# zxhuang1698/ZeroShape

Measured on AMD Instinct MI355X. Metric: sdf_query_points_per_sec_vox128, higher is better.
Workload: dtype f16x3

## Files before the change

zeroshape_amd/build.py:

```python
import hashlib
import os
import subprocess
import sys

HERE = os.path.dirname(os.path.abspath(__file__))
CSRC = os.path.join(HERE, "csrc")
INCLUDE = os.path.join(os.path.dirname(HERE), "include")
LIB = os.path.join(HERE, "libzeroshape_hip.so")
OBJDIR = os.path.join(HERE, "csrc", "_obj")

ARCH = "gfx950"
COMMON = ["--offload-arch=" + ARCH, "-O3", "-std=c++17", "-fPIC", "-Wall",
          "-Wno-unused-function", "-I", INCLUDE]
EXTRA = {
    "chamfer.hip": ["-ffp-contract=off", "-fno-slp-vectorize"],
    "chamfer_grid.hip": ["-ffp-contract=off"],
    "pose_search.hip": ["-ffp-contract=off"],
    "sdf_decoder_split.hip": ["-fno-slp-vectorize", "-fno-honor-nans", "-mllvm", "-amdgpu-mfma-vgpr-form"],
    "marching_cubes.hip": ["-ffp-contract=off"],
    "render.hip": ["-ffp-contract=off"],
    "attn_vis.hip": ["-ffp-contract=off"],
    "seen_mesh.hip": ["-ffp-contract=off"],
    "mesh_weld.hip": ["-ffp-contract=off"],
    "field_normals.hip": ["-ffp-contract=off"],
    "mesh_components.hip": ["-ffp-contract=off"],
    "mesh_colors.hip": ["-ffp-contract=off"],
    "mesh_smooth.hip": ["-ffp-contract=off"],
    "mesh_simplify.hip": ["-ffp-contract=off"],
    "mesh_distance.hip": ["-ffp-contract=off"],
}


def sources():
    return sorted(f for f in os.listdir(CSRC) if f.endswith(".hip"))


def _includes(path, seen):
    import re
    with open(path, "rb") as fh:
        text = fh.read().decode("utf-8", "replace")
    for name in re.findall(r'^\s*#\s*include\s+["<]([^">]+)[">]', text, flags=re.M):
        for base in (os.path.dirname(path), INCLUDE):
            f = os.path.normpath(os.path.join(base, name))
            if os.path.exists(f):
                if f not in seen:
                    seen.append(f)
                    _includes(f, seen)
                break
    return seen


def _stamp(src, flags):
    h = hashlib.sha1()
    h.update(" ".join(os.path.relpath(f, HERE) if os.path.isabs(f) else f for f in flags).encode())
    for f in [src] + sorted(_includes(src, [])):
        with open(f, "rb") as fh:
            h.update(fh.read())
    return h.hexdigest()


def build(force=False, verbose=False):
    hipcc = os.environ.get("HIPCC", "/opt/rocm/bin/hipcc")
    os.makedirs(OBJDIR, exist_ok=True)
    objs, rebuilt = [], False
    for name in sources():
        src = os.path.join(CSRC, name)
        obj = os.path.join(OBJDIR, name[:-4] + ".o")
        flags = COMMON + EXTRA.get(name, [])
        stamp_file = obj + ".stamp"
        stamp = _stamp(src, flags)
        old = open(stamp_file).read() if os.path.exists(stamp_file) else ""
        if force or not os.path.exists(obj) or old != stamp:
            cmd = [hipcc] + flags + ["-c", src, "-o", obj]
            if verbose:
                print(" ".join(cmd), flush=True)
            subprocess.check_call(cmd)
            with open(stamp_file, "w") as fh:
                fh.write(stamp)
            rebuilt = True
        objs.append(obj)
    if rebuilt or not os.path.exists(LIB):
        cmd = [hipcc, "--offload-arch=" + ARCH, "-shared", "-fPIC", "-o", LIB] + objs
        if verbose:
            print(" ".join(cmd), flush=True)
        subprocess.check_call(cmd)
    return LIB


if __name__ == "__main__":
    print(build(force="--force" in sys.argv, verbose="--verbose" in sys.argv or "-v" in sys.argv))
```

zeroshape_amd/csrc/sdf_prologue.hip:

```cpp
#include "zs_common.h"
#include "sdf_layout.h"
#include "../../include/zeroshape_hip.h"

#include <math.h>

namespace {

using namespace zs::lay;

constexpr int ROWS = 4;
constexpr int LIN_THREADS = 256;
constexpr int KMAX = 1024;

__device__ __forceinline__ float wave_sum(float v) {
#pragma unroll
    for (int o = 32; o > 0; o >>= 1) v += __shfl_xor(v, o, 64);
    return v;
}

__device__ __forceinline__ float erf_ref(float x) { return erff(x); }

template <bool LN_IN, bool GELU, bool RESID, bool POS>
__global__ __launch_bounds__(LIN_THREADS) void lat_linear_kernel(
    const float *__restrict__ X, int ldx, size_t x_stride, int K, const float *__restrict__ Wt,
    const float *__restrict__ bias, int N, const float *__restrict__ ln_g,
    const float *__restrict__ ln_b, const float *__restrict__ resid, int ldr, size_t r_stride,
    const float *__restrict__ pos, float *__restrict__ Y, int ldy, size_t y_stride, int rows) {
    __shared__ float xs[ROWS][KMAX];
    const int img = blockIdx.z;
    const int r0 = blockIdx.x * ROWS;
    const int n = blockIdx.y * LIN_THREADS + threadIdx.x;
    X += (size_t)img * x_stride;
    Y += (size_t)img * y_stride;

    for (int i = threadIdx.x; i < ROWS * K; i += LIN_THREADS) {
        const int r = i / K, k = i - r * K;
        const int rr = min(r0 + r, rows - 1);
        xs[r][k] = X[(size_t)rr * ldx + k];
    }
    __syncthreads();
    if (LN_IN) {
        const int w = threadIdx.x >> 6, lane = threadIdx.x & 63;
        float v[4], s = 0.f;
#pragma unroll
        for (int j = 0; j < 4; j++) {
            v[j] = xs[w][lane + 64 * j];
            s += v[j];
        }
        const float mean = wave_sum(s) * (1.0f / 256.0f);
        float q = 0.f;
#pragma unroll
        for (int j = 0; j < 4; j++) {
            const float d = v[j] - mean;
            q = fmaf(d, d, q);
        }
        const float rstd = 1.0f / sqrtf(wave_sum(q) * (1.0f / 256.0f) + 1e-6f);
#pragma unroll
        for (int j = 0; j < 4; j++) {
            const int k = lane + 64 * j;
            xs[w][k] = fmaf((v[j] - mean) * rstd, ln_g[k], ln_b[k]);
        }
        __syncthreads();
    }
    float acc[ROWS];
#pragma unroll
    for (int r = 0; r < ROWS; r++) acc[r] = 0.f;
    for (int k0 = 0; k0 < K; k0 += 16) {
        float w[16];
#pragma unroll
        for (int j = 0; j < 16; j++) w[j] = Wt[(size_t)(k0 + j) * N + n];
#pragma unroll
        for (int j = 0; j < 16; j++)
#pragma unroll
            for (int r = 0; r < ROWS; r++) acc[r] = fmaf(xs[r][k0 + j], w[j], acc[r]);
    }
    const float b = bias[n];
#pragma unroll
    for (int r = 0; r < ROWS; r++) {
        const int row = r0 + r;
        if (row >= rows) break;
        float v = acc[r] + b;
        if (POS) v += pos[(size_t)row * N + n];
        if (GELU) v = 0.5f * v * (1.0f + erf_ref(v * 0.70710678118654752440f));
        if (RESID) v += resid[(size_t)img * r_stride + (size_t)row * ldr + n];
        Y[(size_t)row * ldy + n] = v;
    }
}

__global__ __launch_bounds__(256) void lat_self_attn_kernel(const float *__restrict__ qkv,
                                                            size_t stride, float *__restrict__ out,
                                                            size_t out_stride) {
    __shared__ float ks[L][HD];
    __shared__ float vs[L][HD];
    const int hd = blockIdx.x, img = blockIdx.y;
    qkv += (size_t)img * stride;
    out += (size_t)img * out_stride;
    for (int i = threadIdx.x; i < L * HD; i += 256) {
        const int r = i / HD, d = i - r * HD;
        ks[r][d] = qkv[(size_t)r * (3 * C) + C + hd * HD + d];
        vs[r][d] = qkv[(size_t)r * (3 * C) + 2 * C + hd * HD + d];
    }
    __syncthreads();
    const int i = threadIdx.x;
    if (i >= L) return;
    float q[HD], o[HD];
#pragma unroll
    for (int d = 0; d < HD; d++) {
        q[d] = qkv[(size_t)i * (3 * C) + hd * HD + d];
        o[d] = 0.f;
    }
    const float scale = 0.17677669529663688110f;
    float m = -INFINITY, z = 0.f;
    for (int j = 0; j < L; j++) {
        float s = 0.f;
#pragma unroll
        for (int d = 0; d < HD; d++) s = fmaf(q[d], ks[j][d], s);
        s *= scale;
        const float mn = fmaxf(m, s);
        const float a = expf(m - mn), p = expf(s - mn);
        z = fmaf(z, a, p);
#pragma unroll
        for (int d = 0; d < HD; d++) o[d] = fmaf(p, vs[j][d], o[d] * a);
        m = mn;
    }
    const float inv = 1.0f / z;
#pragma unroll
    for (int d = 0; d < HD; d++) out[(size_t)i * C + hd * HD + d] = o[d] * inv;
}

__global__ __launch_bounds__(256) void pack_kv_kernel(const float *__restrict__ scratch,
                                                      size_t scratch_stride,
                                                      float *__restrict__ programs,
                                                      size_t program_stride) {
    const int img = blockIdx.y;
    const int e = blockIdx.x * 256 + threadIdx.x;
    const int lane = e & 63;
    const int r = (e >> 6) & 15;
    const int which = (e >> 10) & 1;
    int t = e >> 11;
    const int lt = t % LT;
    t /= LT;
    const int hd = t & 7;
    const int blk = t >> 3;
    if (blk >= BLOCKS) return;
    const float *sc = scratch + (size_t)img * scratch_stride;
    const int rw = (r & 3) + 8 * (r >> 2) + 4 * (lane >> 5);
    const int lrow = 32 * lt + (which == 0 ? (lane & 31) : rw);
    const int dim = which == 0 ? rw : (lane & 31);
    float val = 0.f;
    if (lrow < L) {
        if (blk == 0)
            val = sc[S_QKV0 + (size_t)lrow * (3 * C) + (1 + which) * C + hd * HD + dim];
        else
            val = sc[S_KV1 + (size_t)lrow * (2 * C) + which * C + hd * HD + dim];
    }
    const int group = blk * G_BLOCK + hd * G_HEAD + G_QKV_HEAD + lt * 8 + which * 4 + (r >> 2);
    programs[(size_t)img * program_stride + (size_t)group * GROUP_FLOATS + lane * 4 + (r & 3)] = val;
}

template <bool LN_IN, bool GELU, bool RESID, bool POS>
void launch_linear(hipStream_t s, int batch, const float *X, int ldx, size_t x_stride, int K,
                   const float *Wt, const float *bias, int N, const float *g, const float *b,
                   const float *resid, int ldr, size_t r_stride, const float *pos, float *Y, int ldy,
                   size_t y_stride) {
    dim3 grid((L + ROWS - 1) / ROWS, N / LIN_THREADS, batch);
    hipLaunchKernelGGL((lat_linear_kernel<LN_IN, GELU, RESID, POS>), grid, dim3(LIN_THREADS), 0, s, X,
                       ldx, x_stride, K, Wt, bias, N, g, b, resid, ldr, r_stride, pos, Y, ldy,
                       y_stride, L);
}

}

__global__ __launch_bounds__(256) void verdict_stats_kernel(const float *__restrict__ got, const float *__restrict__ want, int m,
                                                            float band, float tol, float tol_occ, float *__restrict__ stats,
                                                            int *__restrict__ flags) {
    __shared__ float red[4][256];
    __shared__ int redi[2][256];
    const int b = blockIdx.x, t = threadIdx.x;
    const float *g = got + (size_t)b * m, *w = want + (size_t)b * m;
    float mx = 0.f, sum = 0.f, mw = 0.f, mo = 0.f;
    int flips = 0, bad = 0;
    for (int i = t; i < m; i += 256) {
        const float x = g[i], y = w[i];
        if (!isfinite(x) || !isfinite(y)) bad = 1;
        const float d = fabsf(x - y);
        mx = fmaxf(mx, d);
        sum += d;
        mw = fmaxf(mw, fabsf(y));
        mo = fmaxf(mo, fabsf(1.0f / (1.0f + expf(-x)) - 1.0f / (1.0f + expf(-y))));
        flips += ((x > 0.f) != (y > 0.f)) && fabsf(y) >= band;
    }
    red[0][t] = mx; red[1][t] = sum; red[2][t] = mw; red[3][t] = mo;
    redi[0][t] = flips; redi[1][t] = bad;
    __syncthreads();
    for (int o = 128; o > 0; o >>= 1) {
        if (t < o) {
            red[0][t] = fmaxf(red[0][t], red[0][t + o]);
            red[1][t] += red[1][t + o];
            red[2][t] = fmaxf(red[2][t], red[2][t + o]);
            red[3][t] = fmaxf(red[3][t], red[3][t + o]);
            redi[0][t] += redi[0][t + o];
            redi[1][t] |= redi[1][t + o];
        }
        __syncthreads();
    }
    if (t == 0) {
        const bool finite = redi[1][0] == 0;
        const float nan = __builtin_bit_cast(float, 0x7fc00000u);
        float *o = stats + (size_t)b * 5;
        o[0] = finite ? red[0][0] : nan;
        o[1] = finite ? red[1][0] / (float)m : nan;
        o[2] = finite ? red[2][0] : nan;
        o[3] = finite ? red[3][0] : nan;
        o[4] = (float)redi[0][0];
        if (flags) {
            flags[2 * b] = (finite && red[0][0] <= tol) ? 0 : 1;
            flags[2 * b + 1] = (finite && red[3][0] <= tol_occ && redi[0][0] == 0) ? 0 : 1;
        }
    }
}

extern "C" int zs_sdf_verdict_stats(const float *got, const float *want, int batch, int m, float flip_band, float tol,
                                    float tol_occ, float *stats, int *flags, void *stream) {
    if (batch < 0 || batch > 65535 || m <= 0) {
        zs::set_err("zs_sdf_verdict_stats: bad size (batch=%d m=%d)", batch, m);
        return 0;
    }
    if (batch == 0) return 1;
    if (!got || !want || !stats) {
        zs::set_err("zs_sdf_verdict_stats: null pointer");
        return 0;
    }
    hipLaunchKernelGGL(verdict_stats_kernel, dim3(batch), dim3(256), 0, static_cast<hipStream_t>(stream), got, want, m, flip_band,
                       tol, tol_occ, stats, flags);
    return zs::check_launch("zs_sdf_verdict_stats") ? 1 : 0;
}

extern "C" size_t zs_sdf_prologue_scratch_bytes(void) { return (size_t)SCRATCH_FLOATS * sizeof(float); }

extern "C" int zs_sdf_prologue(void *programs, size_t program_stride_bytes, const float *lat_params,
                               const float *latent_depth, int batch, void *scratch, void *stream) {
    return zs_sdf_prologue_ex(programs, program_stride_bytes, lat_params, latent_depth, batch, scratch, 0, stream);
}

extern "C" int zs_sdf_prologue_ex(void *programs, size_t program_stride_bytes, const float *lat_params,
                                  const float *latent_depth, int batch, void *scratch, int flags, void *stream) {
    if (flags & ~ZS_SDF_POS_PERLAYER) {
        zs::set_err("zs_sdf_prologue_ex: unknown flags 0x%x", flags);
        return 0;
    }
    if (batch < 0) {
        zs::set_err("zs_sdf_prologue: negative batch %d", batch);
        return 0;
    }
    if (batch == 0) return 1;
    if (!programs || !lat_params || !latent_depth || !scratch) {
        zs::set_err("zs_sdf_prologue: null pointer");
        return 0;
    }
    if (program_stride_bytes % 16 != 0 || program_stride_bytes < zs_sdf_program_bytes()) {
        zs::set_err("zs_sdf_prologue: bad program stride %zu", program_stride_bytes);
        return 0;
    }
    if (batch > 65535) {
        zs::set_err("zs_sdf_prologue: batch %d > 65535", batch);
        return 0;
    }
    hipStream_t s = static_cast<hipStream_t>(stream);
    const float *P = lat_params;
    float *sc = static_cast<float *>(scratch);
    const size_t ss = SCRATCH_FLOATS;
    launch_linear<false, false, false, true>(s, batch, latent_depth, C, (size_t)L * C, C, P + LQ_WLP,
                                             P + LQ_BLP, C, nullptr, nullptr, nullptr, 0, 0,
                                             P + LQ_POS, sc + S_LAT, C, ss);
    launch_linear<true, false, false, false>(s, batch, sc + S_LAT, C, ss, C, P + LQ_WQKV0,
                                             P + LQ_BQKV0, 3 * C, P + LQ_LN1G0, P + LQ_LN1B0, nullptr,
                                             0, 0, nullptr, sc + S_QKV0, 3 * C, ss);
    hipLaunchKernelGGL(lat_self_attn_kernel, dim3(HEADS, batch), dim3(256), 0, s, sc + S_QKV0, ss,
                       sc + S_ATT, ss);
    launch_linear<false, false, true, false>(s, batch, sc + S_ATT, C, ss, C, P + LQ_WPROJ0,
                                             P + LQ_BPROJ0, C, nullptr, nullptr, sc + S_LAT, C, ss,
                                             nullptr, sc + S_X1, C, ss);
    launch_linear<true, true, false, false>(s, batch, sc + S_X1, C, ss, C, P + LQ_W1, P + LQ_B1, HID,
                                            P + LQ_LN2G0, P + LQ_LN2B0, nullptr, 0, 0, nullptr,
                                            sc + S_HID, HID, ss);
    if (flags & ZS_SDF_POS_PERLAYER)
        launch_linear<false, false, true, true>(s, batch, sc + S_HID, HID, ss, HID, P + LQ_W2, P + LQ_B2,
                                                C, nullptr, nullptr, sc + S_X1, C, ss, P + LQ_POS,
                                                sc + S_X2, C, ss);
    else
        launch_linear<false, false, true, false>(s, batch, sc + S_HID, HID, ss, HID, P + LQ_W2, P + LQ_B2,
                                                 C, nullptr, nullptr, sc + S_X1, C, ss, nullptr,
                                                 sc + S_X2, C, ss);
    launch_linear<true, false, false, false>(s, batch, sc + S_X2, C, ss, C, P + LQ_WKV1, P + LQ_BKV1,
                                             2 * C, P + LQ_LN1G1, P + LQ_LN1B1, nullptr, 0, 0, nullptr,
                                             sc + S_KV1, 2 * C, ss);
    const int elems = BLOCKS * HEADS * LT * 2 * 16 * 64;
    hipLaunchKernelGGL(pack_kv_kernel, dim3((elems + 255) / 256, batch), dim3(256), 0, s, sc, ss,
                       static_cast<float *>(programs), program_stride_bytes / sizeof(float));
    return zs::check_launch("zs_sdf_prologue") ? 1 : 0;
}
```

Before: 82.39 million.

## Restructure prologue linear and self-attention kernels for more parallelism and prefetch

The latent linear kernel drops to 64 threads per block, stages inputs with vectorized 16-byte loads, and streams weights through a software-pipelined ring of buffer loads separated by scheduling barriers. The self-attention kernel is re-parallelized so each block handles 8 query rows with one thread per (row, dim), computing scores, a parallel-prefix online-softmax rescale, and the weighted sum in separate shared-memory phases. The intent is to cut prologue latency through better occupancy and hidden weight-load latency. The risks are extra shared-memory passes, the assumption that K is a multiple of 256 in the staging, and the prologue being a small share of the query throughput metric.

```diff
diff --git a/zeroshape_amd/build.py b/zeroshape_amd/build.py
--- a/zeroshape_amd/build.py
+++ b/zeroshape_amd/build.py
@@ -17,6 +17,7 @@
     "chamfer_grid.hip": ["-ffp-contract=off"],
     "pose_search.hip": ["-ffp-contract=off"],
     "sdf_decoder_split.hip": ["-fno-slp-vectorize", "-fno-honor-nans", "-mllvm", "-amdgpu-mfma-vgpr-form"],
+    "sdf_prologue.hip": ["-fno-slp-vectorize"],
     "marching_cubes.hip": ["-ffp-contract=off"],
     "render.hip": ["-ffp-contract=off"],
     "attn_vis.hip": ["-ffp-contract=off"],
diff --git a/zeroshape_amd/csrc/sdf_prologue.hip b/zeroshape_amd/csrc/sdf_prologue.hip
--- a/zeroshape_amd/csrc/sdf_prologue.hip
+++ b/zeroshape_amd/csrc/sdf_prologue.hip
@@ -7,9 +7,18 @@
 namespace {
 
 using namespace zs::lay;
+typedef float f32x4 __attribute__((ext_vector_type(4)));
 
 constexpr int ROWS = 4;
+#ifdef ZS_PROLOGUE_PARENT
 constexpr int LIN_THREADS = 256;
+#else
+constexpr int LIN_THREADS = 64;
+constexpr int LIN_PF_LOADS = 16;
+constexpr int LIN_PF_GROUPS = 2;
+constexpr int LIN_W_AUX = 16;
+constexpr int LIN_PF_UNROLL = 16;
+#endif
 constexpr int KMAX = 1024;
 
 __device__ __forceinline__ float wave_sum(float v) {
@@ -26,21 +35,41 @@
     const float *__restrict__ bias, int N, const float *__restrict__ ln_g,
     const float *__restrict__ ln_b, const float *__restrict__ resid, int ldr, size_t r_stride,
     const float *__restrict__ pos, float *__restrict__ Y, int ldy, size_t y_stride, int rows) {
-    __shared__ float xs[ROWS][KMAX];
+    __shared__ __attribute__((aligned(16))) float xs[ROWS][KMAX];
     const int img = blockIdx.z;
     const int r0 = blockIdx.x * ROWS;
     const int n = blockIdx.y * LIN_THREADS + threadIdx.x;
     X += (size_t)img * x_stride;
     Y += (size_t)img * y_stride;
 
+#ifndef ZS_PROLOGUE_PARENT
+    {
+        static_assert(LIN_THREADS == 64 && KMAX % 256 == 0, "lat_linear_kernel's staging");
+        f32x4 v[ROWS][KMAX / 256];
+#pragma unroll
+        for (int r = 0; r < ROWS; r++) {
+            const f32x4 *row = reinterpret_cast<const f32x4 *>(X + (size_t)min(r0 + r, rows - 1) * ldx);
+#pragma unroll
+            for (int c = 0; c < KMAX / 256; c++)
+                if (c * 256 < K) v[r][c] = row[c * 64 + threadIdx.x];
+        }
+#pragma unroll
+        for (int r = 0; r < ROWS; r++)
+#pragma unroll
+            for (int c = 0; c < KMAX / 256; c++)
+                if (c * 256 < K) *reinterpret_cast<f32x4 *>(&xs[r][c * 256 + 4 * threadIdx.x]) = v[r][c];
+    }
+#else
     for (int i = threadIdx.x; i < ROWS * K; i += LIN_THREADS) {
         const int r = i / K, k = i - r * K;
         const int rr = min(r0 + r, rows - 1);
         xs[r][k] = X[(size_t)rr * ldx + k];
     }
+#endif
     __syncthreads();
     if (LN_IN) {
-        const int w = threadIdx.x >> 6, lane = threadIdx.x & 63;
+        const int lane = threadIdx.x & 63;
+      for (int w = threadIdx.x >> 6; w < ROWS; w += LIN_THREADS / 64) {
         float v[4], s = 0.f;
 #pragma unroll
         for (int j = 0; j < 4; j++) {
@@ -60,11 +89,38 @@
             const int k = lane + 64 * j;
             xs[w][k] = fmaf((v[j] - mean) * rstd, ln_g[k], ln_b[k]);
         }
+      }
         __syncthreads();
     }
     float acc[ROWS];
 #pragma unroll
     for (int r = 0; r < ROWS; r++) acc[r] = 0.f;
+#ifndef ZS_PROLOGUE_PARENT
+    constexpr int PG = LIN_PF_LOADS, PN = LIN_PF_GROUPS, PU = LIN_PF_UNROLL;
+    static_assert(PU % PN == 0 && PN >= 2 && KMAX % (PU * PG) == 0, "the ring's slots must line up from trip to trip");
+    const __amdgpu_buffer_rsrc_t wrsrc = __builtin_amdgcn_make_buffer_rsrc(const_cast<float *>(Wt), 0, K * N * 4, 0x00020000);
+    const int nb = n * 4;
+    auto wld = [&](int k) { return __builtin_bit_cast(float, __builtin_amdgcn_raw_buffer_load_b32(wrsrc, nb, k * N * 4, LIN_W_AUX)); };
+    float w[PN][PG];
+#pragma unroll
+    for (int g = 0; g < PN - 1; g++)
+#pragma unroll
+        for (int j = 0; j < PG; j++) w[g][j] = wld(g * PG + j);
+    for (int k0 = 0; k0 < K; k0 += PU * PG) {
+#pragma unroll
+        for (int g = 0; g < PU; g++) {
+            const int kn = min(k0 + (g + PN - 1) * PG, K - PG);
+#pragma unroll
+            for (int j = 0; j < PG; j++) w[(g + PN - 1) % PN][j] = wld(kn + j);
+            __builtin_amdgcn_sched_barrier(0);
+#pragma unroll
+            for (int j = 0; j < PG; j++)
+#pragma unroll
+                for (int r = 0; r < ROWS; r++) acc[r] = fmaf(xs[r][k0 + g * PG + j], w[g % PN][j], acc[r]);
+            __builtin_amdgcn_sched_barrier(0);
+        }
+    }
+#else
     for (int k0 = 0; k0 < K; k0 += 16) {
         float w[16];
 #pragma unroll
@@ -74,6 +130,7 @@
 #pragma unroll
             for (int r = 0; r < ROWS; r++) acc[r] = fmaf(xs[r][k0 + j], w[j], acc[r]);
     }
+#endif
     const float b = bias[n];
 #pragma unroll
     for (int r = 0; r < ROWS; r++) {
@@ -87,6 +144,100 @@
     }
 }
 
+#ifndef ZS_PROLOGUE_PARENT
+constexpr int ATT_ROWS = 8;
+constexpr int ATT_THREADS = ATT_ROWS * HD;
+constexpr int ATT_KV_LD = HD + 4;
+constexpr int ATT_LP = (L + 3) / 4 * 4;
+static_assert(ATT_THREADS == 256 && (L - 1) % 4 == 0 && ATT_LP <= 4 * 64 && ATT_ROWS % 4 == 0, "lat_self_attn_kernel's thread maps");
+__global__ __launch_bounds__(ATT_THREADS) void lat_self_attn_kernel(const float *__restrict__ qkv,
+                                                                    size_t stride, float *__restrict__ out,
+                                                                    size_t out_stride) {
+    __shared__ __attribute__((aligned(16))) float ks[L][ATT_KV_LD];
+    __shared__ __attribute__((aligned(16))) float vs[L][ATT_KV_LD];
+    __shared__ __attribute__((aligned(16))) float qs[ATT_ROWS][HD];
+    __shared__ __attribute__((aligned(16))) float ts[ATT_ROWS][ATT_LP];
+    __shared__ __attribute__((aligned(16))) float as[ATT_ROWS][ATT_LP];
+    __shared__ __attribute__((aligned(16))) float ps[ATT_ROWS][ATT_LP];
+    const int hd = blockIdx.x, i0 = blockIdx.y * ATT_ROWS, img = blockIdx.z, t = threadIdx.x;
+    qkv += (size_t)img * stride;
+    out += (size_t)img * out_stride;
+    for (int e = t; e < L * (HD / 4); e += ATT_THREADS) {
+        const int r = e / (HD / 4), c = e - r * (HD / 4);
+        const float *row = qkv + (size_t)r * (3 * C) + hd * HD + 4 * c;
+        *reinterpret_cast<f32x4 *>(&ks[r][4 * c]) = *reinterpret_cast<const f32x4 *>(row + C);
+        *reinterpret_cast<f32x4 *>(&vs[r][4 * c]) = *reinterpret_cast<const f32x4 *>(row + 2 * C);
+    }
+    qs[t / HD][t % HD] = qkv[(size_t)min(i0 + t / HD, L - 1) * (3 * C) + hd * HD + t % HD];
+    __syncthreads();
+    {
+        const int i = t % ATT_ROWS, jb = t / ATT_ROWS;
+        float q[HD];
+#pragma unroll
+        for (int d = 0; d < HD; d++) q[d] = qs[i][d];
+#pragma unroll
+        for (int it = 0; it < (L + 31) / 32; it++) {
+            const int j = jb + 32 * it, jc = min(j, L - 1);
+            float s = 0.f;
+#pragma unroll
+            for (int d = 0; d < HD; d++) s = fmaf(q[d], ks[jc][d], s);
+            if (j < L) ts[i][j] = s;
+        }
+    }
+    __syncthreads();
+    const float scale = 0.17677669529663688110f;
+    {
+        const int lane = t & 63;
+        for (int i = t >> 6; i < ATT_ROWS; i += ATT_THREADS / 64) {
+            float sum[4], s[4], before[4], top = -INFINITY;
+#pragma unroll
+            for (int c = 0; c < 4; c++) {
+                const int j = 4 * lane + c;
+                sum[c] = j < L ? ts[i][j] : 0.f;
+                s[c] = sum[c] * scale;
+                before[c] = top;
+                if (j < L) top = fmaxf(top, s[c]);
+            }
+#pragma unroll
+            for (int o = 1; o < 64; o <<= 1) {
+                const float up = __shfl_up(top, o, 64);
+                if (lane >= o) top = fmaxf(top, up);
+            }
+            float lower = __shfl_up(top, 1, 64);
+            if (lane == 0) lower = -INFINITY;
+#pragma unroll
+            for (int c = 0; c < 4; c++) {
+                const int j = 4 * lane + c;
+                const float m = fmaxf(lower, before[c]);
+                const float mn = fmaxf(m, s[c]);
+                const float a = expf(m - mn), p = expf(fmaf(sum[c], scale, -mn));
+                if (j < L) {
+                    as[i][j] = a;
+                    ps[i][j] = p;
+                }
+            }
+        }
+    }
+    __syncthreads();
+    {
+        const int i = t / HD, d = t % HD;
+        float o = 0.f, z = 0.f;
+        for (int j0 = 0; j0 < L - 1; j0 += 4) {
+            const f32x4 a4 = *reinterpret_cast<const f32x4 *>(&as[i][j0]), p4 = *reinterpret_cast<const f32x4 *>(&ps[i][j0]);
+#pragma unroll
+            for (int c = 0; c < 4; c++) {
+                z = fmaf(z, a4[c], p4[c]);
+                o = fmaf(p4[c], vs[j0 + c][d], o * a4[c]);
+            }
+        }
+        const float a = as[i][L - 1], p = ps[i][L - 1];
+        z = fmaf(z, a, p);
+        o = fmaf(p, vs[L - 1][d], o * a);
+        const float inv = 1.0f / z;
+        if (i0 + i < L) out[(size_t)(i0 + i) * C + hd * HD + d] = o * inv;
+    }
+}
+#else
 __global__ __launch_bounds__(256) void lat_self_attn_kernel(const float *__restrict__ qkv,
                                                             size_t stride, float *__restrict__ out,
                                                             size_t out_stride) {
@@ -127,6 +278,7 @@
 #pragma unroll
     for (int d = 0; d < HD; d++) out[(size_t)i * C + hd * HD + d] = o[d] * inv;
 }
+#endif
 
 __global__ __launch_bounds__(256) void pack_kv_kernel(const float *__restrict__ scratch,
                                                       size_t scratch_stride,
@@ -276,8 +428,13 @@
     launch_linear<true, false, false, false>(s, batch, sc + S_LAT, C, ss, C, P + LQ_WQKV0,
                                              P + LQ_BQKV0, 3 * C, P + LQ_LN1G0, P + LQ_LN1B0, nullptr,
                                              0, 0, nullptr, sc + S_QKV0, 3 * C, ss);
+#ifndef ZS_PROLOGUE_PARENT
+    hipLaunchKernelGGL(lat_self_attn_kernel, dim3(HEADS, (L + ATT_ROWS - 1) / ATT_ROWS, batch), dim3(ATT_THREADS), 0, s,
+                       sc + S_QKV0, ss, sc + S_ATT, ss);
+#else
     hipLaunchKernelGGL(lat_self_attn_kernel, dim3(HEADS, batch), dim3(256), 0, s, sc + S_QKV0, ss,
                        sc + S_ATT, ss);
+#endif
     launch_linear<false, false, true, false>(s, batch, sc + S_ATT, C, ss, C, P + LQ_WPROJ0,
                                              P + LQ_BPROJ0, C, nullptr, nullptr, sc + S_LAT, C, ss,
                                              nullptr, sc + S_X1, C, ss);
```

Measured after the change: 82.61 million (median of 6 runs). About the same (+0.3%).
